# jzebedee/deltaq

Hardware: AMD Instinct MI355X
Metric: MB of text suffix-sorted per second (bit-exact SA) (higher is better)
Workload: dtype u8 text / u64 keys / int32 SA; 1 GPU; 256 MiB uniform-random bytes per GPU (splitmix64 seed 0x5EED0003+rank), int32 SA; bytes_per_gpu=268435456, residency=text and SA resident in HBM, rounds_after_initial_sort=1

## Files before the change

deltaq_amd/csrc/dq_flags.h:

```cpp
#pragma once

#include <algorithm>
#include <cstdint>
#include <cstdlib>
#include <cstring>
#include <optional>
#include <string>

namespace dq {

struct Flags {
    bool debug = false;
    std::optional<int> trace;
    std::optional<int> hip_device;
    std::optional<int> numa_bind;
    std::optional<std::string> fault;
    std::optional<int> small_n;
    std::optional<int> no_many;
    std::optional<int> mid_many_min;
    std::optional<int> no_large_many;
    std::optional<int> large_many_min;
    std::optional<int> no_diff_many;
    std::optional<int> no_diff_mid_many;
    std::optional<int> diff_mid_many_min;
    std::optional<int> no_diff_large;
    std::optional<int> diff_large_min;
    std::optional<int> diff_large_table;
    std::optional<int> no_index_many;
    std::optional<int> index_many_min;
    std::optional<int> index_many_threads;
    std::optional<int> no_index_large;
    std::optional<int> index_large_min;
    std::optional<int> no_check_many;
    std::optional<int> no_bwt_many;
    std::optional<int> no_mtf_many;
    std::optional<int> no_huff_many;
    std::optional<int> mtf_short_max;
    std::optional<int> unbz2_one_start;
    bool no_list_buffers = false;
    bool text_copy = false;
    bool assume_doubled = false;
    bool no_twins = false;
    bool no_period_hint = false;
    std::optional<int> xcd_group;
    std::optional<int> packed;
    std::optional<int> key_bytes;
    std::optional<int> coded;
    std::optional<int> split;
    bool no_bucket = false;
    std::optional<int> bucket;
    std::optional<int> bucket_keybits;
    std::optional<int> bucket_ext;
    std::optional<int> bucket_tile;
    std::optional<int> bucket_slots;
    bool old_first_pass = false;
    bool no_fused_ties = false;
    std::optional<int> sparse;
    std::optional<int> binned_isa;
    bool no_binned_isa = false;
    std::optional<int> runs;
    bool no_small = false;
    bool no_wide_small = false;
    bool no_first_small = false;
    std::optional<int> mid_groups;
    bool no_l_shift = false;
    bool no_upd_words = false;
    std::optional<int> upd_bin;
    std::optional<int> upd_bin_min;
    std::optional<int> upd_window;
    std::optional<int> chain_steps;
    bool no_chain = false;
    bool force_rshift = false;
    std::optional<int> tail_max;
    std::optional<int> pair_chains;
    std::optional<int> pair_chains_min;
    std::optional<int> pair_maxg;
    std::optional<int> late_runs_min;
    bool no_late_runs = false;
    std::optional<int> run_period;
    bool search_wave = false;
    std::optional<int> search_ptab;
    bool no_wave_windows = false;
    bool no_poll = false;
    bool no_second_stage = false;
    std::optional<int> win_min;
    std::optional<int> win_second;
    std::optional<int> walk_on;
// ... 44 lines not shown
    f.no_diff_mid_many = num("DQ_NO_DIFF_MID_MANY", 0, 1);
    f.diff_mid_many_min = num("DQ_DIFF_MID_MANY_MIN", 1);
    f.no_diff_large = num("DQ_NO_DIFF_LARGE", 0, 1);
    f.diff_large_min = num("DQ_DIFF_LARGE_MIN", 1);
    f.diff_large_table = num("DQ_DIFF_LARGE_TABLE", 0, 1);
    f.no_index_many = num("DQ_NO_INDEX_MANY", 0, 1);
    f.index_many_min = num("DQ_INDEX_MANY_MIN", 1);
    f.index_many_threads = num("DQ_INDEX_MANY_THREADS");
    f.no_index_large = num("DQ_NO_INDEX_LARGE", 0, 1);
    f.index_large_min = num("DQ_INDEX_LARGE_MIN", 1);
    f.no_check_many = num("DQ_NO_CHECK_MANY", 0, 1);
    f.no_bwt_many = num("DQ_NO_BWT_MANY", 0, 1);
    f.no_mtf_many = num("DQ_NO_MTF_MANY", 0, 1);
    f.no_huff_many = num("DQ_NO_HUFF_MANY", 0, 1);
    f.mtf_short_max = num("DQ_MTF_SHORT_MAX", 0);
    f.unbz2_one_start = num("DQ_UNBZ2_ONE_START", 0, 1);
    f.no_list_buffers = on("DQ_NO_LIST_BUFFERS");
    f.text_copy = on("DQ_TEXT_COPY");
    f.assume_doubled = on("DQ_ASSUME_DOUBLED");
    f.no_twins = on("DQ_NO_TWINS");
    f.no_period_hint = on("DQ_NO_PERIOD_HINT");

    f.xcd_group = num("DQ_XCD_GROUP", 0, 64);
    f.packed = num("DQ_PACKED");
    f.key_bytes = num("DQ_KEY_BYTES", 1, 8);
    f.coded = num("DQ_CODED");
    f.split = num("DQ_SPLIT");
    f.no_bucket = on("DQ_NO_BUCKET");
    f.bucket = num("DQ_BUCKET");
    f.bucket_keybits = num("DQ_BUCKET_KEYBITS");
    f.bucket_ext = num("DQ_BUCKET_EXT");
    f.bucket_tile = num("DQ_BUCKET_TILE", 0, 1);
    f.bucket_slots = num("DQ_BUCKET_SLOTS", 0, 1);
    f.old_first_pass = on("DQ_OLD_FIRST_PASS");
    f.no_fused_ties = on("DQ_NO_FUSED_TIES");
    f.sparse = num("DQ_SPARSE");
    f.binned_isa = num("DQ_BINNED_ISA");
    f.no_binned_isa = on("DQ_NO_BINNED_ISA");
    f.runs = num("DQ_RUNS");

    f.no_small = on("DQ_NO_SMALL");
    f.no_wide_small = on("DQ_NO_WIDE_SMALL");
    f.no_first_small = on("DQ_NO_FIRST_SMALL");
    f.mid_groups = num("DQ_MID_GROUPS");
    f.no_l_shift = on("DQ_NO_L_SHIFT");
    f.no_upd_words = on("DQ_NO_UPD_WORDS");
    f.upd_bin = num("DQ_UPD_BIN", 0, 2);
    f.upd_bin_min = num("DQ_UPD_BIN_MIN", 1);
    f.upd_window = num("DQ_UPD_WINDOW");
    f.chain_steps = num("DQ_CHAIN_STEPS");
    f.no_chain = on("DQ_NO_CHAIN");
    f.force_rshift = on("DQ_FORCE_RSHIFT");

    f.tail_max = num("DQ_TAIL_MAX", 0);
    f.pair_chains = num("DQ_PAIR_CHAINS");
    f.pair_chains_min = num("DQ_PAIR_CHAINS_MIN", 1);
    f.pair_maxg = num("DQ_PAIR_MAXG", 2);
    f.late_runs_min = num("DQ_LATE_RUNS_MIN", 1);
    f.no_late_runs = on("DQ_NO_LATE_RUNS");
    f.run_period = num("DQ_RUN_PERIOD", 1);

    f.search_wave = on("DQ_SEARCH_WAVE");
    f.search_ptab = num("DQ_SEARCH_PTAB");
    f.no_wave_windows = on("DQ_NO_WAVE_WINDOWS");
    f.no_poll = on("DQ_NO_POLL");
    f.no_second_stage = on("DQ_NO_SECOND_STAGE");
// ... 78 lines not shown
```

deltaq_amd/csrc/dq_round0.h:

```cpp
#pragma once
#include "dq_sort_passes.h"
#include "dq_alpha_code.h"
#include "dq_ties.h"
#include "dq_bucket_sort.h"
#include "dq_xcd_rank.h"
#include "dq_slot_rank.h"

namespace dq {
namespace {

constexpr int64_t kSgShortList = 1 << 20;
inline int mid_group_cap(int64_t list_len)
{
    if (const std::optional<int> g = flags().mid_groups) {
        return *g >= 1024 ? 1024 : *g >= 512 ? 512 : *g >= 256 ? 256 : 0;
    }
    return list_len >= kSgShortList ? 512 : 1024;
}
inline bool small_round_usable(int64_t n, int64_t mm, bool third_list_buffer)
{
    const Flags &F = flags();
    return !F.no_small && n < (1ll << 32) && (mm * 2 <= n || (third_list_buffer && !F.no_wide_small));
}

// ... 67 lines not shown
        int blocks = (int)std::min<int64_t>(1024, ((n >> 4) + kBlock - 1) / kBlock + 1);
        unsigned long long *xcd_hist = n >= kRound0MinN ? reinterpret_cast<unsigned long long *>(w.bytehist + kXcdHistAt) : nullptr;
        if (xcd_hist) blocks = (blocks + kXcds - 1) / kXcds * kXcds;
        HIP_TRY(hipMemsetAsync(w.bytehist, 0, (size_t)(kXcdHistAt + (xcd_hist ? kXcds * kRadixSize : 0)) * 8, L.st));
        LAUNCH(L, DQ_K_TEXT_HIST, n, n,
               hipLaunchKernelGGL(text_hist_kernel, dim3(blocks + 1), dim3(kBlock), 0, L.st,
                                  text_src ? text_src : (const uint8_t *)w.text, n, reinterpret_cast<unsigned long long *>(w.bytehist),
                                  reinterpret_cast<unsigned long long *>(w.bytehist + 256), text_src ? w.text : (uint8_t *)nullptr,
                                  xcd_hist));
        HIP_TRY(hipMemcpyAsync(c.pinned, w.bytehist, (256 + 10) * 8, hipMemcpyDeviceToHost, L.st));
        HIP_TRY(hipEventRecord(c.readback, L.st));
        constexpr int kEarlyPasses = 3;
        DQ_TRY(prepare_status<IdxT>(L, w, n, kEarlyPasses));
        if (n >= kRound0MinN) HIP_TRY(hipMemsetAsync(w.Vb, 0, (size_t)(tie_words() + 1) * 8, L.st));
        HIP_TRY(hipEventSynchronize(c.readback));
        const Flags &F = flags();
        s = TextStats(c.pinned, n);
        ib = s.ib;
        k = choose_key_bytes(s, F);
        DQ_TRY(prepare_status<IdxT>(L, w, n, k.kb, kEarlyPasses));
        bool hist_deferred = false;
        if (coded_keys_tried(s, F, k)) {
            AlphaCode code;
            if (build_alpha_code(s.hist, &code) && (code.avg_len <= kCodedMaxAvgLen || F.coded)) {
                uint16_t *stage = reinterpret_cast<uint16_t *>(c.pinned + 512);
                memcpy(stage, code.tab, sizeof(code.tab));
                HIP_TRY(hipMemcpyAsync(w.codetab, stage, sizeof(code.tab), hipMemcpyHostToDevice, L.st));
                coded = true;
                hist_deferred = split_round0_wanted(n, k, (int)wb, F);
                if (F.trace) fprintf(stderr, "[dq] coded round 0: %d symbols, %.2f bits per byte\n", code.sigma, code.avg_len);
            }
        }
        if (hist_deferred) return DQ_OK;
        return digit_tables(k.kb, coded);
    }

    int passes(int &cur, uint32_t *ebits = nullptr, uint64_t *seam_tab = nullptr)
    {
        const int kb = k.kb;
        if (k.packed) {
            DQ_TRY(rank_pass<IdxT, kTextPacked>(L, w, text64(), (const IdxT *)nullptr, K[1], (IdxT *)nullptr, n, 0, kb, ib));
            cur = 1;
            for (int p = 1; p < kb; ++p) {
                if (p == kb - 1 && ebits)
                    DQ_TRY(rank_pass<IdxT, kKeysLastTies>(L, w, K[cur], (const IdxT *)nullptr, (uint64_t *)nullptr, d_sa, n, p,
                                                          kb, ib, ebits, seam_tab));
                else if (p == kb - 1)
                    DQ_TRY(rank_pass<IdxT, kKeysLast>(L, w, K[cur], (const IdxT *)nullptr, K[cur ^ 1], d_sa, n, p, kb, ib));
                else
                    DQ_TRY(rank_pass<IdxT, kKeys>(L, w, K[cur], (const IdxT *)nullptr, K[cur ^ 1], (IdxT *)nullptr, n, p, kb, ib));
                cur ^= 1;
            }
            return DQ_OK;
        }
        DQ_TRY(with_bool(coded, [&](auto kCoded) -> int {
            return rank_pass<IdxT, kText, decltype(kCoded)::value>(L, w, text64(), (const IdxT *)nullptr, K[1], V[1], n, 0, kb);
        }));
        cur = 1;
        for (int p = 1; p < kb; ++p) {
            DQ_TRY(rank_pass<IdxT, kPairs>(L, w, K[cur], V[cur], K[cur ^ 1], V[cur ^ 1], n, p, kb));
            cur ^= 1;
        }
        return DQ_OK;
    }

    int collect_ties(uint32_t *ebits, const uint64_t *seam_tab, uint64_t *act_rank, bool *overflow, uint64_t *fin_rank,
                     bool seams = true, int64_t h_fin = -1)
    {
        using Cfg = RankCfg<IdxT, kKeysLastTies>;
        using CfgS = RankCfg<IdxT, kKeysLastTies, true>;
        const int64_t tile_keys = small_tiles(n) ? CfgS::kThreads * CfgS::kItems : Cfg::kThreads * Cfg::kItems;
        const int64_t ntiles = (n + tile_keys - 1) / tile_keys;
        const int pass = k.kb - 1;
        char *area = w.ctl_status + (size_t)pass * w.ctl_status_stride;
        const int64_t *dofs = w.digit_offset + pass * kRadixSize;
        TieCounters *ctr = reinterpret_cast<TieCounters *>(w.totals + 6);
        if (seams) {
            HIP_TRY(hipMemsetAsync(ctr, 0, sizeof(TieCounters), L.st));
            const unsigned sg = (unsigned)((ntiles * kRadixSize + kBlock - 1) / kBlock);
            DQ_TRY(with_status_word(n, [&](auto word) -> int {
                LAUNCH(L, DQ_K_TIE_SEAM, ntiles * kRadixSize, ntiles * kRadixSize * (16 + (int64_t)sizeof(uint64_t)),
                       hipLaunchKernelGGL(tie_seam_kernel<decltype(word)>, dim3(sg), dim3(kBlock), 0, L.st, seam_tab, ntiles, ib, dofs,
                                          reinterpret_cast<const decltype(word) *>(area + 256), ebits));
                return DQ_OK;
            }));
        }
        LAUNCH(L, DQ_K_TIE_COLLECT, n, n / 8,
               hipLaunchKernelGGL(tie_collect_kernel<IdxT>, dim3((unsigned)((tie_words() + kTieThreads - 1) / kTieThreads)),
                                  dim3(kTieThreads), 0, L.st, reinterpret_cast<const uint64_t *>(ebits), tie_words(), n, (const IdxT *)d_sa,
                                  act_rank, w.Va, ctr));
        unsigned long long *left_over = reinterpret_cast<unsigned long long *>(w.totals + 3);
        o.fin_cap = n / 8;
        LAUNCH(L, DQ_K_SMALL_FINISH, o.fin_cap, 0,
               hipLaunchKernelGGL((small_group_finish_kernel<IdxT, 8, 32>),
                                  dim3((unsigned)std::min<int64_t>((o.fin_cap + kFinishThreads - 1) / kFinishThreads, 256 * 16)),
                                  dim3(kFinishThreads), 0, L.st, (const uint64_t *)act_rank, (const IdxT *)w.Va, (const uint8_t *)w.text,
                                  o.fin_cap, n, h_fin >= 0 ? h_fin : (int64_t)k.kb, d_sa, fin_rank, w.Vb, left_over,
                                  (const unsigned long long *)&ctr->count));
        DQ_TRY(read_totals<IdxT>(L, c, w, 64, "radix look-back timed out (device spin bound hit)"));
        o.m = c.pinned[6];
        *overflow = c.pinned[7] != 0;
// ... 89 lines not shown
        if (b.xcd_pass) {
            if (F.trace) fprintf(stderr, "[dq] XCD-local first pass (n=%lld, eighths of %lld)\n", (long long)n, (long long)xcd_eighth(n));
            if (sizeof(XcdRankCtl) > w.ctl_status_stride) return fail(DQ_ERR_HIP, "status buffer too small");
            LAUNCH(L, DQ_K_RADIX_RANK, n, n * (1 + 8),
                   hipLaunchKernelGGL(xcd_text_rank_kernel, dim3((unsigned)std::min<int64_t>(c.ncu, (n + kXcdTileN - 1) / kXcdTileN)),
                                      dim3(kXcdRankThreads), 0, st, reinterpret_cast<const uint32_t *>(w.text), K[first], n,
                                      ib + lowbits, keybits, ib, (const int64_t *)w.xcd_offset,
                                      reinterpret_cast<XcdRankCtl *>(w.ctl_status)));
        } else {
            DQ_TRY(b.ext ? rank_pass_ext<IdxT, kTextPackedExt>(L, w, text64(), (const uint8_t *)nullptr, K[1], E[1], n, 0, ib, ib + lowbits, keybits)
                       : rank_pass<IdxT, kTextPacked>(L, w, text64(), (const IdxT *)nullptr, K[first], (IdxT *)nullptr, n, 0, kb, ib,
                                                      nullptr, nullptr, ib + lowbits, keybits));
        }
        if (slots) {
            const int groups = resident_groups(&c.slot_rank_groups, (const void *)slot_rank_kernel, kSlotRankThreads, c.dev);
            LAUNCH(L, DQ_K_RADIX_RANK, n, n * 16,
                   hipLaunchKernelGGL(slot_rank_kernel, dim3((unsigned)std::min<int64_t>(groups, (n + kSlotTileN - 1) / kSlotTileN)),
                                      dim3(kSlotRankThreads), 0, st, (const uint64_t *)K[0], K[1], n, ib + lowbits + 8, ib + lowbits,
                                      (const int64_t *)w.digit_offset, (const uint32_t *)slot_base, sctl, bflags));
        }
        for (int p = 1; p < b.bbytes && !slots; ++p) {
            DQ_TRY(b.ext ? rank_pass_ext<IdxT, kKeysExt>(L, w, K[p & 1], E[p & 1], K[(p & 1) ^ 1], E[(p & 1) ^ 1], n, p, ib, ib + lowbits + 8 * p, keybits)
                       : rank_pass<IdxT, kKeys>(L, w, K[p & 1], (const IdxT *)nullptr, K[(p & 1) ^ 1], (IdxT *)nullptr, n, p, kb, ib,
                                                nullptr, nullptr, ib + lowbits + 8 * p, keybits));
        }
        uint64_t *Ks = slots ? K[1] : K[b.bbytes & 1], *Kfree = slots ? K[0] : K[(b.bbytes & 1) ^ 1];
        const uint8_t *Es = b.ext ? E[b.bbytes & 1] : nullptr;
        if (F.trace)
            fprintf(stderr, "[dq] bucket finish: %s geometry, %lld tiles of up to %lld words cut every %lld %s (n=%lld)\n", ft.fine ? "fine" : "coarse",
                    (long long)ft.ntiles, (long long)ft.cap, (long long)(ft.by_id ? ft.g : ft.Cf), ft.by_id ? "buckets" : "words", (long long)n);
        if ((size_t)ft.ntiles + 1 > finish_bounds_entries(n)) return fail(DQ_ERR_HIP, "tile bounds buffer too small");
        if (slots) {
            LAUNCH(L, DQ_K_BUCKET_SORT, ft.ntiles, ft.ntiles * 16,
                   hipLaunchKernelGGL(slot_out_kernel, dim3(1), dim3(kSlotOutThreads), 0, st, sctl->cursor, (uint32_t)b.X, slot_out, bflags));
            auto kernel = bucket_sort_kernel<IdxT, false, BktFine, true>;
            const int groups = resident_groups(&c.bkt_slot_groups[sizeof(IdxT) == 8], (const void *)kernel, BktFine::threads, c.dev);
            LAUNCH(L, DQ_K_BUCKET_SORT, n, n * (8 + wb) + n / 8,
                   hipLaunchKernelGGL(kernel, dim3((unsigned)std::min<int64_t>(ft.ntiles, groups)), dim3(BktFine::threads), 0, st,
                                      (const uint64_t *)Ks, ib, lowbits, (const int64_t *)nullptr, ft.ntiles, d_sa, ebits, bflags,
                                      (const uint8_t *)nullptr, (const uint32_t *)slot_base, (const uint32_t *)sctl->cursor, (const uint32_t *)slot_out));
        } else if (ft.by_id) {
            const int64_t nbuckets = (int64_t)1 << (8 * b.bbytes);
            LAUNCH(L, DQ_K_BUCKET_SORT, ft.ntiles, ft.ntiles * 16 * 8,
                   hipLaunchKernelGGL(bucket_bounds_by_id_kernel, dim3((unsigned)((nbuckets + 1 + kBlock - 1) / kBlock)), dim3(kBlock), 0,
                                      st, (const uint64_t *)Ks, n, ib + lowbits, ft.g, b.X, nbuckets, ft.ntiles, w.bkt_bounds, bflags));
        } else {
            LAUNCH(L, DQ_K_BUCKET_SORT, ft.ntiles, ft.ntiles * 16 * 8,
                   hipLaunchKernelGGL(bucket_bounds_kernel, dim3((unsigned)((ft.ntiles + 1 + kBlock - 1) / kBlock)), dim3(kBlock), 0,
                                      st, (const uint64_t *)Ks, n, ib + lowbits, ft.Cf, b.X, ft.ntiles, w.bkt_bounds, bflags));
        }
        auto finish = [&](auto kExt, auto geometry) -> int {
            using G = decltype(geometry);
            auto kernel = bucket_sort_kernel<IdxT, decltype(kExt)::value, G>;
            const int groups = resident_groups(&c.bkt_groups[ft.fine][b.ext][sizeof(IdxT) == 8], (const void *)kernel, G::threads, c.dev);
            LAUNCH(L, DQ_K_BUCKET_SORT, n, n * ((b.ext ? 9 : 8) + wb) + n / 8,
                   hipLaunchKernelGGL(kernel, dim3((unsigned)std::min<int64_t>(ft.ntiles, groups)), dim3(G::threads), 0, st,
                                      (const uint64_t *)Ks, ib, lowbits, (const int64_t *)w.bkt_bounds, ft.ntiles, d_sa, ebits, bflags, Es,
                                      (const uint32_t *)nullptr, (const uint32_t *)nullptr, (const uint32_t *)nullptr));
            return DQ_OK;
        };
        if (slots) {
        } else if (ft.fine) {
            DQ_TRY(finish(std::false_type{}, BktFine{}));
        } else {
            DQ_TRY(with_bool(b.ext, [&](auto kExt) -> int { return finish(kExt, BktCoarse{}); }));
        }
        if (b.ext && F.trace) fprintf(stderr, "[dq] bucketed round 0 with %d + 8 key bits per suffix (n=%lld)\n", keybits, (long long)n);
        bool overflow = false;
        DQ_TRY(collect_ties(ebits, nullptr, Kfree, &overflow, Ks, false, b.hb));
        if (overflow) {
            if (F.trace) fprintf(stderr, "[dq] bucketed round 0 gave up (n=%lld): plain digit passes\n", (long long)n);
            DQ_TRY(prepare_status<IdxT>(L, w, n, kMaxPasses));
            HIP_TRY(hipMemsetAsync(w.Vb, 0, (size_t)(tie_words() + 1) * 8, st));
            HIP_TRY(hipMemsetAsync(w.totals, 0, 64, st));
            o.m = 0; o.fin_cap = 0; o.fin_left = 0;
            return digit_tables(kb, false);
        }
        o.fin_done = o.m <= o.fin_cap;
        o.Kr[0] = Kfree; o.Kr[1] = Ks;
        o.h = b.hb;
        o.shallow_ties = true;
        *done = true;
        return DQ_OK;
    }

    int split(bool *done)
    {
        *done = false;
        if constexpr (sizeof(IdxT) != 4) {
            return DQ_OK;
        } else {
            if (!w.sp_top || !w.X || !w.RL) return DQ_OK;
            const int64_t cap = std::min<int64_t>(kFinCap, (n + 2) / (kSplitBuckets / 2));
            if (cap < 2) return DQ_OK;
            const uint32_t *t32 = reinterpret_cast<const uint32_t *>(w.text);
            const uint16_t *ctab = (const uint16_t *)w.codetab;
            uint64_t *Ks[2] = {K[0], w.X};
            IdxT *Vs[2] = {w.Vb, w.Xs};
            const int64_t ovf_cap = (n / 2) & ~(int64_t)1;
            uint64_t *ovf_k[2] = {reinterpret_cast<uint64_t *>(w.ISA), K[0]};
            IdxT *ovf_v[2] = {reinterpret_cast<IdxT *>(w.RL), w.Vb};
            const Flags &F = flags();
            const bool dbg = F.trace.value_or(0) >= 2;
            auto phase = [&](const char *what) -> int {
                if (!dbg) return DQ_OK;
                HIP_TRY(hipStreamSynchronize(st));
                fprintf(stderr, "[dq] split round 0: %s done\n", what);
                return DQ_OK;
            };
            const unsigned sgrid = (unsigned)((kSplitSample + kBlock - 1) / kBlock);
            DQ_TRY(with_bool(coded, [&](auto kCoded) -> int {
                LAUNCH(L, DQ_K_SPLIT_AUX, kSplitSample, kSplitSample * ((coded ? 20 : 12) + 8),
// ... 162 lines not shown
```

deltaq_amd/csrc/dq_sa_kernels.h:

```cpp
#pragma once
#include "dq_runs.h"
#include "dq_device_utils.h"

namespace dq {

template <typename IdxT>
__global__ __launch_bounds__(kBlock) void gather_key2_kernel(uint64_t *__restrict__ comp,
                                                             const IdxT *__restrict__ suf,
                                                             const IdxT *__restrict__ ISA,
                                                             int64_t m, int64_t n, int64_t h, int kbits,
                                                             int rshift = 0,
                                                             const uint32_t *__restrict__ RL = nullptr ,
                                                             const uint8_t *__restrict__ text = nullptr, int run_order = 0)
{
    for (int64_t j = (int64_t)blockIdx.x * kBlock + threadIdx.x; j < m;
         j += (int64_t)gridDim.x * kBlock) {
        const int64_t s = (int64_t)suf[j];
        int64_t off = h;
        uint64_t k2 = 0;
        bool keyed = false;
        if (RL) {
            const uint32_t r = RL[s];
            if (run_order) { k2 = (int64_t)r >= h ? (uint64_t)run_order_key(text, n, s, r, run_order) : 0ull; keyed = true; }
            else if ((int64_t)r > h) off = (int64_t)r;
        }
        if (!keyed) {
            const int64_t q = s + off;
            k2 = q < n ? (uint64_t)((int64_t)ISA[q] + h) : (off > h ? 0ull : (uint64_t)(n - 1 - s));
        }
        comp[j] = ((comp[j] >> rshift) << kbits) | k2;
    }
}

// ... 33 lines not shown
    if (m_dev) {
        const unsigned long long real = m_dev[0];
        if (real > (unsigned long long)m || m_dev[1] != 0) return;
        m = (int64_t)real;
    }
    __shared__ uint32_t wave_tot[kFinishThreads / kWave];
    __shared__ unsigned long long s_base;
    const int lane = lane_id();
    const int w = threadIdx.x >> 6;
    for (int64_t j0 = (int64_t)blockIdx.x * kFinishThreads; j0 < m; j0 += (int64_t)gridDim.x * kFinishThreads) {
    const int64_t j = j0 + threadIdx.x;

    uint32_t emit = 0;
    uint64_t r = 0;
    int g = 1;
    bool head = false;
    if (j < m) {
        r = rank[j];
        int left = 0, right = 0;
#pragma unroll
        for (int i = 1; i <= kMaxG; ++i)
            if (left == i - 1 && j - i >= 0 && rank[j - i] == r) left = i;
#pragma unroll
        for (int i = 1; i <= kMaxG; ++i)
            if (right == i - 1 && j + i < m && rank[j + i] == r) right = i;
        g = left + right + 1;
        if (g > kMaxG) emit = 1;
        else head = left == 0;
    }
    int64_t s[kMaxG];
    if (head) {
#pragma unroll
        for (int i = 0; i < kMaxG; ++i) s[i] = i < g ? (int64_t)suf[j + i] : 0;
        static_assert(kMaxLen % 8 == 0, "whole words");
        typedef uint64_t u64_any __attribute__((aligned(1)));
        auto cmp = [&](int64_t a, int64_t b) -> int {
            const int64_t pa = a + h, pb = b + h;
            uint64_t wa[kMaxLen / 8], wbv[kMaxLen / 8];
#pragma unroll
            for (int k = 0; k < kMaxLen / 8; ++k) {
                wa[k] = *reinterpret_cast<const u64_any *>(text + pa + 8 * k);
                wbv[k] = *reinterpret_cast<const u64_any *>(text + pb + 8 * k);
            }
            int d = kMaxLen;
            bool a_less = false;
#pragma unroll
            for (int k = kMaxLen / 8 - 1; k >= 0; --k) {
                const uint64_t x = __builtin_bswap64(wa[k]), y = __builtin_bswap64(wbv[k]);
                if (x != y) { d = 8 * k + (__builtin_clzll(x ^ y) >> 3); a_less = x < y; }
            }
            const int64_t la = n - pa, lb = n - pb;
            const int64_t lim = la < lb ? (la < kMaxLen ? la : kMaxLen) : (lb < kMaxLen ? lb : kMaxLen);
            if (d < lim) return a_less ? -1 : 1;
            if (lim < kMaxLen) return la < lb ? -1 : 1;
            return 0;
        };
        bool decided = true;
        if (g == 2) {
            const int c = cmp(s[0], s[1]);
            if (c == 0) decided = false;
            if (c > 0) { const int64_t t = s[0]; s[0] = s[1]; s[1] = t; }
        } else
#pragma unroll
        for (int pass = 0; pass < kMaxG - 1; ++pass) {
#pragma unroll
            for (int i = 0; i < kMaxG - 1; ++i) {
                if (i + 1 < g && i < g - 1 - pass) {
                    const int c = cmp(s[i], s[i + 1]);
                    if (c == 0) decided = false;
                    if (c > 0) { const int64_t t = s[i]; s[i] = s[i + 1]; s[i + 1] = t; }
                }
            }
        }
        if (decided) {
#pragma unroll
            for (int i = 0; i < kMaxG; ++i)
                if (i < g) SA[(int64_t)r + i] = (IdxT)s[i];
        } else {
            emit = (uint32_t)g;
        }
    }
    const uint32_t incl = wave_incl_sum(emit);
    if (lane == kWave - 1) wave_tot[w] = incl;
    __syncthreads();
    uint32_t off = incl - emit, tot = 0;
#pragma unroll
    for (int k = 0; k < kFinishThreads / kWave; ++k) {
        const uint32_t c = wave_tot[k];
        if (k < w) off += c;
// ... 23 lines not shown
        const int64_t p = (int64_t)((__int128)i * (m - 1) / samples);
        tie = (keys[p] >> kshift) == (keys[p + 1] >> kshift);
    }
    const uint64_t b = __ballot(tie);
    if (lane_id() == 0 && b) atomicAdd((unsigned long long *)count, (unsigned long long)__popcll(b));
}

template <typename IdxT>
__global__ __launch_bounds__(kBlock) void isa_from_sa_kernel(const IdxT *__restrict__ SA,
                                                             IdxT *__restrict__ ISA, int64_t n)
{
    for (int64_t p = (int64_t)blockIdx.x * kBlock + threadIdx.x; p < n; p += (int64_t)gridDim.x * kBlock)
        ISA[SA[p]] = (IdxT)p;
}

template <typename IdxT>
__global__ __launch_bounds__(kBlock) void sa_words_kernel(const IdxT *__restrict__ SA, int64_t n, int ib,
                                                          uint64_t *__restrict__ words)
{
    for (int64_t p = (int64_t)blockIdx.x * kBlock + threadIdx.x; p < n; p += (int64_t)gridDim.x * kBlock)
        words[p] = ((uint64_t)p << ib) | (uint64_t)SA[p];
}

template <typename IdxT>
__global__ __launch_bounds__(kBlock) void isa_scatter_kernel(const uint64_t *__restrict__ rank,
                                                             const IdxT *__restrict__ suf,
                                                             IdxT *__restrict__ ISA, int64_t m)
{
    for (int64_t j = (int64_t)blockIdx.x * kBlock + threadIdx.x; j < m; j += (int64_t)gridDim.x * kBlock)
        ISA[suf[j]] = (IdxT)rank[j];
}

}
```

deltaq_amd/csrc/dq_slot_rank.h:

```cpp
#pragma once
#include "dq_bucket_sort.h"
#include "dq_xcd_rank.h"

namespace dq {

constexpr int kSlotBuckets = 1 << 16;

struct SlotRankCtl {
    uint32_t ticket[kXcds];
    uint32_t pad[64 - kXcds];
    uint32_t cursor[kSlotBuckets];
};

static __global__ __launch_bounds__(kBlock) void slot_plan_kernel(const int64_t *__restrict__ bytehist, int64_t X,
                                                           uint32_t *__restrict__ slot_base )
{
    __shared__ int tmp[kWavesPerBlock];
    __shared__ int s_rank, s_present;
    const int d = threadIdx.x, A = blockIdx.x;
    const int pa = bytehist[d] > 0 ? 1 : 0, pb = (pa || d == 0) ? 1 : 0;
    int na, nb;
    const int ra = block_excl_sum(pa, tmp, &na);
    __syncthreads();
    const int rb = block_excl_sum(pb, tmp, &nb);
    if (A == kRadixSize) {
        if (d == 0) slot_base[kSlotBuckets] = (uint32_t)(X * na * nb);
        return;
    }
    if (d == A) { s_rank = ra; s_present = pa; }
    __syncthreads();
    slot_base[A * kRadixSize + d] = (uint32_t)(X * ((int64_t)s_rank * nb + (s_present ? rb : 0)));
}

constexpr int kSlotOutThreads = 1024;
static __global__ __launch_bounds__(kSlotOutThreads) void slot_out_kernel(uint32_t *__restrict__ count , uint32_t X,
                                                                   uint32_t *__restrict__ out ,
                                                                   BucketFlags *__restrict__ flags)
{
    constexpr int kPer = kSlotBuckets / kSlotOutThreads, kVec = kPer / 4;
    __shared__ uint32_t wtot[kSlotOutThreads / kWave];
    const int tid = threadIdx.x, lane = lane_id(), wv = tid >> 6;
    uint4 *cv = reinterpret_cast<uint4 *>(count) + tid * kVec;
    uint4 c[kVec];
#pragma unroll
    for (int i = 0; i < kVec; ++i) c[i] = cv[i];
    uint32_t sum = 0, mx = 0;
#pragma unroll
    for (int i = 0; i < kVec; ++i) {
        mx = max(max(max(c[i].x, c[i].y), max(c[i].z, c[i].w)), mx);
        c[i].x = min(c[i].x, X); c[i].y = min(c[i].y, X); c[i].z = min(c[i].z, X); c[i].w = min(c[i].w, X);
        sum += c[i].x + c[i].y + c[i].z + c[i].w;
    }
    if (mx > X) {
        atomicOr(&flags->overflow, 2ull);
#pragma unroll
        for (int i = 0; i < kVec; ++i) cv[i] = c[i];
    }
    const uint32_t incl = wave_incl_sum(sum);
    if (lane == kWave - 1) wtot[wv] = incl;
    __syncthreads();
    uint32_t run = incl - sum;
    for (int i = 0; i < wv; ++i) run += wtot[i];
    uint4 *ov = reinterpret_cast<uint4 *>(out) + tid * kVec;
#pragma unroll
    for (int i = 0; i < kVec; ++i) {
        uint4 o;
        o.x = run; run += c[i].x;
        o.y = run; run += c[i].y;
        o.z = run; run += c[i].z;
        o.w = run; run += c[i].w;
        ov[i] = o;
    }
    if (tid == kSlotOutThreads - 1) out[kSlotBuckets] = run;
}

#ifdef DQ_SLOT_PHASE_TIMING
__device__ long long *g_slot_ts = nullptr;
__device__ unsigned int g_slot_ts_next = 0;
#define DQ_SLOT_PHASE(i) do { if (threadIdx.x == 0 && g_slot_ts) g_slot_ts[(long long)ts_row * 8 + (i)] = clock64(); } while (0)
#else
#define DQ_SLOT_PHASE(i) do { } while (0)
#endif

constexpr int kSlotRankThreads = 1024;
constexpr int kSlotRankItems = 12;
constexpr int kSlotTileN = kSlotRankThreads * kSlotRankItems;

static __global__ __launch_bounds__(kSlotRankThreads, 1) void slot_rank_kernel(
    const uint64_t *__restrict__ kin , uint64_t *__restrict__ wout, int64_t n,
    int shift , int bshift ,
    const int64_t *__restrict__ region , const uint32_t *__restrict__ slot_base ,
    SlotRankCtl *__restrict__ ctl, BucketFlags *__restrict__ flags)
{
    constexpr int kThreads = kSlotRankThreads, kItems = kSlotRankItems, kTileN = kSlotTileN;
    constexpr int kPerXcd = kRadixSize / kXcds;
    __shared__ __attribute__((aligned(16))) uint64_t exch[kTileN];
    __shared__ uint32_t cnt[kRadixSize];
    __shared__ uint32_t tile_base[kRadixSize];
    __shared__ uint32_t gofs[kRadixSize];
    __shared__ uint32_t glim[kRadixSize];
    __shared__ uint32_t wtmp[kRadixSize / kWave];
    __shared__ uint32_t r_lo[kRadixSize], r_hi[kRadixSize], r_tiles[kRadixSize];
    __shared__ uint32_t xs[kXcds][kPerXcd + 1];
    __shared__ uint32_t s_lo, s_cnt;

    const int tid = threadIdx.x;
// ... 142 lines not shown
```

deltaq_amd/csrc/dq_ties.h:

```cpp
#pragma once
#include "dq_onesweep.h"

namespace dq {

constexpr int kTieMaxRun = 4096;
constexpr int kTieThreads = 1024;

template <typename StatusT>
__global__ __launch_bounds__(kBlock) void tie_seam_kernel(const uint64_t *__restrict__ seam_tab, int64_t ntiles,
                                                          int ib, const int64_t *__restrict__ digit_offset,
                                                          const StatusT *__restrict__ status,
                                                          uint32_t *__restrict__ ebits)
{
    using SB = StatusBits<StatusT>;
    const int64_t idx = (int64_t)blockIdx.x * kBlock + threadIdx.x;
    if (idx >= ntiles * kRadixSize) return;
    const int64_t t = idx / kRadixSize;
    const int d = (int)(idx % kRadixSize);
    const uint64_t first = seam_tab[idx * 2];
    if (first == kSeamEmpty || t == 0) return;
    int64_t tp = t - 1;
    while (tp >= 0 && seam_tab[(tp * kRadixSize + d) * 2] == kSeamEmpty) --tp;
    if (tp < 0) return;
    const uint64_t last = seam_tab[(tp * kRadixSize + d) * 2 + 1];
    if ((last >> ib) != (first >> ib)) return;
    const int64_t o = digit_offset[d] + (int64_t)(status[(t - 1) * kRadixSize + d] & SB::kMask);
    atomicOr(&ebits[(uint64_t)o >> 5], 1u << ((uint32_t)o & 31u));
}

struct TieCounters {
    unsigned long long count;
    unsigned long long overflow;
};

// ... 69 lines not shown
    uint64_t todo = __ballot(cnt != 0);
    const uint64_t lbit = 1ull << lane;
    while (todo) {
        const int j = __builtin_ctzll(todo);
        todo &= todo - 1;
        const uint64_t own_j = ((uint64_t)(uint32_t)__builtin_amdgcn_readlane((int)(uint32_t)(own >> 32), j) << 32) |
                               (uint32_t)__builtin_amdgcn_readlane((int)(uint32_t)own, j);
        const uint64_t E_j = ((uint64_t)(uint32_t)__builtin_amdgcn_readlane((int)(uint32_t)(E >> 32), j) << 32) |
                             (uint32_t)__builtin_amdgcn_readlane((int)(uint32_t)E, j);
        const int64_t out_j = (int64_t)(((uint64_t)(uint32_t)__builtin_amdgcn_readlane((int)(uint32_t)((uint64_t)out >> 32), j) << 32) |
                                        (uint32_t)__builtin_amdgcn_readlane((int)(uint32_t)(uint64_t)out, j));
        const uint32_t tail_j = (uint32_t)__builtin_amdgcn_readlane((int)tail, j);
        const int64_t p0 = (i - lane + j) * 64;
        if (own_j & lbit) {
            const uint64_t below = lbit - 1;
            const int64_t p = p0 + lane;
            const int64_t head = (E_j & lbit) ? p0 + (63 - __builtin_clzll(~E_j & below)) : p;
            const int64_t o = out_j + __popcll(own_j & below);
            act_rank[o] = (uint64_t)head;
            act_suf[o] = SA[p];
        }
        if (tail_j) {
            const int64_t head = p0 + (63 - __builtin_clzll(~E_j));
            const int64_t o0 = out_j + __popcll(own_j);
            for (uint32_t k = (uint32_t)lane; k < tail_j; k += kWave) {
                act_rank[o0 + k] = (uint64_t)head;
                act_suf[o0 + k] = SA[p0 + 64 + k];
            }
        }
    }
    (void)n;
}

}
```

Before: 91260 MB/s.

## Settle small tie groups in place from boundary bits in bucketed round 0

Adds a tie_settle kernel that scans the equality bitmap, resolves small tied groups (up to 8) directly in the SA by comparing a 32-byte text window, and lists only unresolved groups for later rounds. It becomes the default when slot bucketing is used, replacing the collect-everything path so the follow-up round processes far fewer suffixes. The slot_out prefix kernel is parallelised across 256 blocks and clamped to digit offsets, and digit tables are skipped when the bucketed plan applies. This risks extra random text reads and more complex overflow handling.

```diff
diff --git a/deltaq_amd/csrc/dq_flags.h b/deltaq_amd/csrc/dq_flags.h
--- a/deltaq_amd/csrc/dq_flags.h
+++ b/deltaq_amd/csrc/dq_flags.h
@@ -53,6 +53,7 @@
     std::optional<int> bucket_ext;
     std::optional<int> bucket_tile;
     std::optional<int> bucket_slots;
+    std::optional<int> tie_settle;
     bool old_first_pass = false;
     bool no_fused_ties = false;
     std::optional<int> sparse;
@@ -163,6 +164,7 @@
     f.bucket_ext = num("DQ_BUCKET_EXT");
     f.bucket_tile = num("DQ_BUCKET_TILE", 0, 1);
     f.bucket_slots = num("DQ_BUCKET_SLOTS", 0, 1);
+    f.tie_settle = num("DQ_TIE_SETTLE", 0, 1);
     f.old_first_pass = on("DQ_OLD_FIRST_PASS");
     f.no_fused_ties = on("DQ_NO_FUSED_TIES");
     f.sparse = num("DQ_SPARSE");
diff --git a/deltaq_amd/csrc/dq_round0.h b/deltaq_amd/csrc/dq_round0.h
--- a/deltaq_amd/csrc/dq_round0.h
+++ b/deltaq_amd/csrc/dq_round0.h
@@ -123,6 +123,7 @@
             }
         }
         if (hist_deferred) return DQ_OK;
+        if (!coded && plan_bucketed(s, F, k, coded, (int)wb).applies) return DQ_OK;
         return digit_tables(k.kb, coded);
     }
 
@@ -156,8 +157,28 @@
     }
 
     int collect_ties(uint32_t *ebits, const uint64_t *seam_tab, uint64_t *act_rank, bool *overflow, uint64_t *fin_rank,
-                     bool seams = true, int64_t h_fin = -1)
-    {
+                     bool seams = true, int64_t h_fin = -1, bool settle = false)
+    {
+        if (settle) {
+            TieCounters *tctr = reinterpret_cast<TieCounters *>(w.totals + 6);
+            unsigned long long *listed = reinterpret_cast<unsigned long long *>(w.totals + 3);
+            const int64_t tile = (int64_t)kSettleThreads * kSettleWords;
+            const int64_t groups = std::min<int64_t>((tie_words() + tile - 1) / tile, (int64_t)std::max(c.ncu, 1) * 6);
+            o.fin_cap = n;
+            LAUNCH(L, DQ_K_TIE_COLLECT, n, n / 8,
+                   hipLaunchKernelGGL(tie_settle_kernel<IdxT>, dim3((unsigned)groups), dim3(kSettleThreads), 0, L.st,
+                                      reinterpret_cast<const uint64_t *>(ebits), tie_words(), n, d_sa, (const uint8_t *)w.text,
+                                      h_fin >= 0 ? h_fin : (int64_t)k.kb, act_rank, w.Va, o.fin_cap, tctr, listed));
+            DQ_TRY(read_totals<IdxT>(L, c, w, 64, "radix look-back timed out (device spin bound hit)"));
+            o.m = c.pinned[6];
+            o.fin_left = c.pinned[3];
+            *overflow = c.pinned[7] != 0 || o.fin_left > o.fin_cap;
+            if (flags().trace)
+                fprintf(stderr, "[dq] ties settled from their bits: %lld tied suffixes, %lld of them listed (n=%lld)\n", (long long)o.m,
+                        (long long)o.fin_left, (long long)n);
+            if (*overflow && flags().trace) fprintf(stderr, "[dq] tie / bucket overflow flags: %lld\n", (long long)c.pinned[7]);
+            return DQ_OK;
+        }
         using Cfg = RankCfg<IdxT, kKeysLastTies>;
         using CfgS = RankCfg<IdxT, kKeysLastTies, true>;
         const int64_t tile_keys = small_tiles(n) ? CfgS::kThreads * CfgS::kItems : Cfg::kThreads * Cfg::kItems;
@@ -313,7 +334,8 @@
         if ((size_t)ft.ntiles + 1 > finish_bounds_entries(n)) return fail(DQ_ERR_HIP, "tile bounds buffer too small");
         if (slots) {
             LAUNCH(L, DQ_K_BUCKET_SORT, ft.ntiles, ft.ntiles * 16,
-                   hipLaunchKernelGGL(slot_out_kernel, dim3(1), dim3(kSlotOutThreads), 0, st, sctl->cursor, (uint32_t)b.X, slot_out, bflags));
+                   hipLaunchKernelGGL(slot_out_kernel, dim3(kRadixSize), dim3(kSlotOutThreads), 0, st, sctl->cursor, (uint32_t)b.X,
+                                      (const int64_t *)(w.digit_offset + kRadixSize) , n, slot_out, bflags));
             auto kernel = bucket_sort_kernel<IdxT, false, BktFine, true>;
             const int groups = resident_groups(&c.bkt_slot_groups[sizeof(IdxT) == 8], (const void *)kernel, BktFine::threads, c.dev);
             LAUNCH(L, DQ_K_BUCKET_SORT, n, n * (8 + wb) + n / 8,
@@ -348,7 +370,8 @@
         }
         if (b.ext && F.trace) fprintf(stderr, "[dq] bucketed round 0 with %d + 8 key bits per suffix (n=%lld)\n", keybits, (long long)n);
         bool overflow = false;
-        DQ_TRY(collect_ties(ebits, nullptr, Kfree, &overflow, Ks, false, b.hb));
+        const bool settle = F.tie_settle.value_or(slots ? 1 : 0) != 0;
+        DQ_TRY(collect_ties(ebits, nullptr, Kfree, &overflow, Ks, false, b.hb, settle));
         if (overflow) {
             if (F.trace) fprintf(stderr, "[dq] bucketed round 0 gave up (n=%lld): plain digit passes\n", (long long)n);
             DQ_TRY(prepare_status<IdxT>(L, w, n, kMaxPasses));
@@ -357,8 +380,12 @@
             o.m = 0; o.fin_cap = 0; o.fin_left = 0;
             return digit_tables(kb, false);
         }
-        o.fin_done = o.m <= o.fin_cap;
+        o.fin_done = settle || o.m <= o.fin_cap;
         o.Kr[0] = Kfree; o.Kr[1] = Ks;
+        if (settle) {
+            o.Kr[0] = Ks; o.Kr[1] = Kfree;
+            o.Vr[0] = w.Vb; o.Vr[1] = w.Va;
+        }
         o.h = b.hb;
         o.shallow_ties = true;
         *done = true;
diff --git a/deltaq_amd/csrc/dq_sa_kernels.h b/deltaq_amd/csrc/dq_sa_kernels.h
--- a/deltaq_amd/csrc/dq_sa_kernels.h
+++ b/deltaq_amd/csrc/dq_sa_kernels.h
@@ -1,4 +1,43 @@
 #pragma once
+#include <stdint.h>
+
+#if defined(__HIPCC__)
+#define DQ_HD __host__ __device__
+#else
+#define DQ_HD
+#endif
+
+namespace dq {
+
+template <int kMaxLen>
+DQ_HD inline int suffix_window_compare(const uint8_t *text, int64_t n, int64_t h, int64_t a, int64_t b)
+{
+    static_assert(kMaxLen % 8 == 0, "whole words");
+    typedef uint64_t u64_any __attribute__((aligned(1), may_alias));
+    const int64_t pa = a + h, pb = b + h;
+    uint64_t wa[kMaxLen / 8], wbv[kMaxLen / 8];
+#pragma unroll
+    for (int k = 0; k < kMaxLen / 8; ++k) {
+        wa[k] = *reinterpret_cast<const u64_any *>(text + pa + 8 * k);
+        wbv[k] = *reinterpret_cast<const u64_any *>(text + pb + 8 * k);
+    }
+    int d = kMaxLen;
+    bool a_less = false;
+#pragma unroll
+    for (int k = kMaxLen / 8 - 1; k >= 0; --k) {
+        const uint64_t x = __builtin_bswap64(wa[k]), y = __builtin_bswap64(wbv[k]);
+        if (x != y) { d = 8 * k + (__builtin_clzll(x ^ y) >> 3); a_less = x < y; }
+    }
+    const int64_t la = n - pa, lb = n - pb;
+    const int64_t lim = la < lb ? (la < kMaxLen ? la : kMaxLen) : (lb < kMaxLen ? lb : kMaxLen);
+    if (d < lim) return a_less ? -1 : 1;
+    if (lim < kMaxLen) return la < lb ? -1 : 1;
+    return 0;
+}
+
+}
+
+#if defined(__HIPCC__)
 #include "dq_runs.h"
 #include "dq_device_utils.h"
 
@@ -98,29 +137,7 @@
     if (head) {
 #pragma unroll
         for (int i = 0; i < kMaxG; ++i) s[i] = i < g ? (int64_t)suf[j + i] : 0;
-        static_assert(kMaxLen % 8 == 0, "whole words");
-        typedef uint64_t u64_any __attribute__((aligned(1)));
-        auto cmp = [&](int64_t a, int64_t b) -> int {
-            const int64_t pa = a + h, pb = b + h;
-            uint64_t wa[kMaxLen / 8], wbv[kMaxLen / 8];
-#pragma unroll
-            for (int k = 0; k < kMaxLen / 8; ++k) {
-                wa[k] = *reinterpret_cast<const u64_any *>(text + pa + 8 * k);
-                wbv[k] = *reinterpret_cast<const u64_any *>(text + pb + 8 * k);
-            }
-            int d = kMaxLen;
-            bool a_less = false;
-#pragma unroll
-            for (int k = kMaxLen / 8 - 1; k >= 0; --k) {
-                const uint64_t x = __builtin_bswap64(wa[k]), y = __builtin_bswap64(wbv[k]);
-                if (x != y) { d = 8 * k + (__builtin_clzll(x ^ y) >> 3); a_less = x < y; }
-            }
-            const int64_t la = n - pa, lb = n - pb;
-            const int64_t lim = la < lb ? (la < kMaxLen ? la : kMaxLen) : (lb < kMaxLen ? lb : kMaxLen);
-            if (d < lim) return a_less ? -1 : 1;
-            if (lim < kMaxLen) return la < lb ? -1 : 1;
-            return 0;
-        };
+        auto cmp = [&](int64_t a, int64_t b) -> int { return suffix_window_compare<kMaxLen>(text, n, h, a, b); };
         bool decided = true;
         if (g == 2) {
             const int c = cmp(s[0], s[1]);
@@ -210,3 +227,4 @@
 }
 
 }
+#endif
diff --git a/deltaq_amd/csrc/dq_slot_rank.h b/deltaq_amd/csrc/dq_slot_rank.h
--- a/deltaq_amd/csrc/dq_slot_rank.h
+++ b/deltaq_amd/csrc/dq_slot_rank.h
@@ -32,46 +32,31 @@
     slot_base[A * kRadixSize + d] = (uint32_t)(X * ((int64_t)s_rank * nb + (s_present ? rb : 0)));
 }
 
-constexpr int kSlotOutThreads = 1024;
+constexpr int kSlotOutThreads = kRadixSize;
 static __global__ __launch_bounds__(kSlotOutThreads) void slot_out_kernel(uint32_t *__restrict__ count , uint32_t X,
+                                                                   const int64_t *__restrict__ first_offset , int64_t n,
                                                                    uint32_t *__restrict__ out ,
                                                                    BucketFlags *__restrict__ flags)
 {
-    constexpr int kPer = kSlotBuckets / kSlotOutThreads, kVec = kPer / 4;
-    __shared__ uint32_t wtot[kSlotOutThreads / kWave];
-    const int tid = threadIdx.x, lane = lane_id(), wv = tid >> 6;
-    uint4 *cv = reinterpret_cast<uint4 *>(count) + tid * kVec;
-    uint4 c[kVec];
-#pragma unroll
-    for (int i = 0; i < kVec; ++i) c[i] = cv[i];
-    uint32_t sum = 0, mx = 0;
-#pragma unroll
-    for (int i = 0; i < kVec; ++i) {
-        mx = max(max(max(c[i].x, c[i].y), max(c[i].z, c[i].w)), mx);
-        c[i].x = min(c[i].x, X); c[i].y = min(c[i].y, X); c[i].z = min(c[i].z, X); c[i].w = min(c[i].w, X);
-        sum += c[i].x + c[i].y + c[i].z + c[i].w;
-    }
-    if (mx > X) {
+    static_assert(kSlotOutThreads == kBlock, "block_excl_sum scans kBlock values");
+    __shared__ uint32_t tmp[kWavesPerBlock];
+    const int A = blockIdx.x, B = threadIdx.x;
+    int64_t lo = first_offset[A], hi = A + 1 < kRadixSize ? first_offset[A + 1] : n;
+    lo = lo < 0 ? 0 : (lo > n ? n : lo);
+    hi = hi < lo ? lo : (hi > n ? n : hi);
+    const uint32_t room = (uint32_t)(hi - lo);
+    const uint32_t raw = count[A * kRadixSize + B];
+    const uint32_t c = min(raw, X);
+    uint32_t total;
+    const uint32_t excl = block_excl_sum(c, tmp, &total);
+    const uint32_t place = min(excl, room);
+    const uint32_t kept = min(c, room - place);
+    if (kept != raw) {
         atomicOr(&flags->overflow, 2ull);
-#pragma unroll
-        for (int i = 0; i < kVec; ++i) cv[i] = c[i];
-    }
-    const uint32_t incl = wave_incl_sum(sum);
-    if (lane == kWave - 1) wtot[wv] = incl;
-    __syncthreads();
-    uint32_t run = incl - sum;
-    for (int i = 0; i < wv; ++i) run += wtot[i];
-    uint4 *ov = reinterpret_cast<uint4 *>(out) + tid * kVec;
-#pragma unroll
-    for (int i = 0; i < kVec; ++i) {
-        uint4 o;
-        o.x = run; run += c[i].x;
-        o.y = run; run += c[i].y;
-        o.z = run; run += c[i].z;
-        o.w = run; run += c[i].w;
-        ov[i] = o;
-    }
-    if (tid == kSlotOutThreads - 1) out[kSlotBuckets] = run;
+        count[A * kRadixSize + B] = kept;
+    }
+    out[A * kRadixSize + B] = (uint32_t)lo + place;
+    if (A == kRadixSize - 1 && B == kRadixSize - 1) out[kSlotBuckets] = (uint32_t)n;
 }
 
 #ifdef DQ_SLOT_PHASE_TIMING
diff --git a/deltaq_amd/csrc/dq_ties.h b/deltaq_amd/csrc/dq_ties.h
--- a/deltaq_amd/csrc/dq_ties.h
+++ b/deltaq_amd/csrc/dq_ties.h
@@ -1,5 +1,6 @@
 #pragma once
 #include "dq_onesweep.h"
+#include "dq_sa_kernels.h"
 
 namespace dq {
 
@@ -135,4 +136,155 @@
     (void)n;
 }
 
-}
+constexpr int kSettleThreads = 256;
+constexpr int kSettleWords = 8;
+constexpr int kSettleQueue = 256;
+constexpr int kSettleMaxG = 8, kSettleLen = 32;
+
+template <typename IdxT>
+__device__ __forceinline__ bool settle_group(IdxT *SA, const uint8_t *__restrict__ text, int64_t n, int64_t h, int64_t head, int g, bool *bad)
+{
+    uint32_t place = 0;
+    bool decided = true;
+#pragma unroll 1
+    for (int i = 0; i + 1 < g && decided; ++i) {
+        const int64_t si = (int64_t)SA[head + i];
+#pragma unroll 1
+        for (int j = i + 1; j < g && decided; ++j) {
+            const int64_t sj = (int64_t)SA[head + j];
+            if (!((uint64_t)si < (uint64_t)n && (uint64_t)sj < (uint64_t)n)) { *bad = true; return false; }
+            const int c = suffix_window_compare<kSettleLen>(text, n, h, si, sj);
+            if (c == 0) decided = false;
+            place += c > 0 ? 1u << (4 * i) : 1u << (4 * j);
+        }
+    }
+    if (!decided) return false;
+    IdxT s[kSettleMaxG];
+#pragma unroll
+    for (int i = 0; i < kSettleMaxG; ++i) s[i] = i < g ? SA[head + i] : (IdxT)0;
+#pragma unroll
+    for (int i = 0; i < kSettleMaxG; ++i)
+        if (i < g) SA[head + (int64_t)((place >> (4 * i)) & 15u)] = s[i];
+    return true;
+}
+
+template <typename IdxT>
+__global__ __launch_bounds__(kSettleThreads, 6) void tie_settle_kernel(
+    const uint64_t *__restrict__ ebits, int64_t nwords, int64_t n, IdxT *SA, const uint8_t *__restrict__ text, int64_t h,
+    uint64_t *__restrict__ list_rank, IdxT *__restrict__ list_suf, int64_t list_cap ,
+    TieCounters *__restrict__ ctr , unsigned long long *__restrict__ list_count )
+{
+    constexpr int kW = kSettleWords, kWaves = kSettleThreads / kWave;
+    constexpr int64_t kWaveWords = (int64_t)kWave * kW, kTile = kWaveWords * kWaves;
+    static_assert(kWaveWords <= 1024 && kSettleQueue % kWave == 0, "a queue entry has 10 bits for the word");
+    if (ctr->overflow != 0 || n < 2) return;
+    __shared__ unsigned long long s_seen;
+    __shared__ uint32_t s_queue[kWaves][kSettleQueue];
+    if (threadIdx.x == 0) s_seen = 0;
+    __syncthreads();
+    const int lane = lane_id(), wv = threadIdx.x >> 6;
+    uint32_t *queue = s_queue[wv];
+    unsigned long long seen = 0;
+    bool over = false;
+    for (int64_t t0 = (int64_t)blockIdx.x * kTile; t0 < nwords; t0 += (int64_t)gridDim.x * kTile) {
+        const int64_t w0 = t0 + (int64_t)wv * kWaveWords;
+        uint32_t P = 0, total = 0;
+        do {
+            uint64_t E[kW];
+            uint32_t first = 0;
+#pragma unroll
+            for (int k = 0; k < kW; ++k) {
+                const int64_t i = w0 + k * kWave + lane;
+                E[k] = i < nwords ? ebits[i] : 0ull;
+            }
+            const int64_t behind = w0 + kWaveWords;
+            const uint32_t last = behind < nwords ? (uint32_t)(ebits[behind] & 1ull) : 0u;
+#pragma unroll
+            for (int k = 0; k < kW; ++k) first |= (uint32_t)(E[k] & 1ull) << k;
+            const uint32_t lane0 = (uint32_t)__builtin_amdgcn_readfirstlane((int)first);
+            const uint32_t up = (uint32_t)__shfl_down((int)first, 1, kWave);
+            const uint32_t goes = lane == kWave - 1 ? ((lane0 >> 1) | (last << (kW - 1))) : up;
+            uint32_t mine = 0;
+#pragma unroll
+            for (int k = 0; k < kW; ++k) mine += (uint32_t)__popcll(((E[k] >> 1) | ((uint64_t)((goes >> k) & 1u) << 63)) & ~E[k]);
+            const uint32_t incl = wave_incl_sum(mine);
+            total = (uint32_t)__shfl((int)incl, kWave - 1, kWave);
+            if (total == 0) break;
+            uint32_t idx = incl - mine;
+#pragma unroll
+            for (int k = 0; k < kW; ++k) {
+                uint64_t heads = ((E[k] >> 1) | ((uint64_t)((goes >> k) & 1u) << 63)) & ~E[k];
+                while (heads != 0) {
+                    const int b = __builtin_ctzll(heads);
+                    heads &= heads - 1;
+                    if (idx - P < (uint32_t)kSettleQueue) {
+                        const int run = b < 63 ? __builtin_ctzll(~(E[k] >> (b + 1))) : 0;
+                        const uint32_t on = (b + run == 63) ? ((goes >> k) & 1u) : 0u;
+                        queue[idx - P] = (uint32_t)(k * kWave + lane) | ((uint32_t)b << 10) | ((uint32_t)(run + 1) << 16) | (on << 23);
+                    }
+                    ++idx;
+                }
+            }
+            __builtin_amdgcn_wave_barrier();
+            const uint32_t cnt = min(total - P, (uint32_t)kSettleQueue);
+            for (uint32_t q0 = 0; q0 < cnt; q0 += kWave) {
+                const uint32_t q = q0 + (uint32_t)lane;
+                const uint32_t e = q < cnt ? queue[q] : 0u;
+                uint32_t g = (e >> 16) & 127u;
+                const int64_t i = w0 + (int64_t)(e & 1023u);
+                const int64_t head = i * 64 + (int64_t)((e >> 10) & 63u);
+                bool bad = false;
+                if ((e >> 23) & 1u) {
+                    uint32_t tail = 0;
+                    for (int64_t j = i + 1;; ++j) {
+                        const uint64_t F = j < nwords ? ebits[j] : 0ull;
+                        const int c = F == ~0ull ? 64 : __builtin_ctzll(~F);
+                        tail += (uint32_t)c;
+                        if (c < 64) break;
+                        if (tail > (uint32_t)kTieMaxRun) { bad = true; break; }
+                    }
+                    g += tail;
+                }
+                if (g != 0 && (bad || head + (int64_t)g > n)) { over = true; g = 0; }
+                const int64_t p = g != 0 ? head : 0;
+                const int64_t s0 = (int64_t)SA[p], s1 = (int64_t)SA[p + 1];
+                if (g != 0 && !((uint64_t)s0 < (uint64_t)n && (uint64_t)s1 < (uint64_t)n)) { over = true; g = 0; }
+                seen += g;
+                const bool small = g != 0 && g <= (uint32_t)kSettleMaxG;
+                const int c = suffix_window_compare<kSettleLen>(text, n, h, small ? s0 : 0, small ? s1 : 0);
+                bool left = g > (uint32_t)kSettleMaxG || (small && c == 0);
+                if (g == 2u) {
+                    if (c > 0) { SA[head] = (IdxT)s1; SA[head + 1] = (IdxT)s0; }
+                } else if (small && c != 0) {
+                    bool bad_entry = false;
+                    if (!settle_group<IdxT>(SA, text, n, h, head, (int)g, &bad_entry)) left = true;
+                    if (bad_entry) { over = true; left = false; }
+                }
+                const uint32_t emit = left ? g : 0u;
+                if (__any(emit != 0)) {
+                    const uint32_t upto = wave_incl_sum(emit);
+                    const uint32_t tot = (uint32_t)__shfl((int)upto, kWave - 1, kWave);
+                    unsigned long long base = 0;
+                    if (lane == kWave - 1) base = atomicAdd(list_count, (unsigned long long)tot);
+                    base = (unsigned long long)__shfl((long long)base, kWave - 1, kWave);
+                    if (emit != 0 && base + tot <= (unsigned long long)list_cap) {
+                        int64_t o = (int64_t)base + (upto - emit);
+                        for (uint32_t j = 0; j < g; ++j, ++o) {
+                            list_rank[o] = (uint64_t)head;
+                            list_suf[o] = SA[head + j];
+                        }
+                    }
+                }
+            }
+            __builtin_amdgcn_wave_barrier();
+            P += (uint32_t)kSettleQueue;
+        } while (P < total);
+    }
+    if (over) atomicOr(&ctr->overflow, 1ull);
+    seen = wave_sum(seen);
+    if (lane == 0 && seen) atomicAdd(&s_seen, seen);
+    __syncthreads();
+    if (threadIdx.x == 0 && s_seen) atomicAdd(&ctr->count, s_seen);
+}
+
+}
```

Result: faster. 93360 MB/s (median of 6 runs) (+2.3%).
